# dome272/Paella

Measured on AMD Instinct MI355X. Metric: images/sec (whole node) + single-image ms, 256x256 @ 8 steps, higher is better.
Workload: dtype f32; 1 GPU; BASELINE configs[1]: Paella 573M-class (stand-in blocks=[4,8,4]) (570.3M params), 32x32 tokens = 256 px, 8 steps, CFG 8.0, CLIP-H-text only (S=4), batch 1 per GPU, + VQGAN f8 decode; denoiser=570m, sample_steps=8, noise=philox, submission=hip-graph replay, world_size_observed=1

## Files before the change

paella_amd/_lib.py:

```python
import ctypes
import os
from ctypes import POINTER, Structure, c_char, c_char_p, c_float, c_int, c_int32, c_int64, c_size_t, c_uint64, c_void_p

_HERE = os.path.dirname(os.path.abspath(__file__))
LIB_PATH = os.path.join(_HERE, "csrc", "libpaella_hip.so")

MAX_LEVELS = 8
MAX_BLOCK_TYPES = 8
ABI_VERSION = 8


class UnetConfig(Structure):
    _fields_ = [
        ("c_in", c_int32), ("c_out", c_int32), ("num_labels", c_int32), ("c_r", c_int32), ("patch_size", c_int32),
        ("c_cond", c_int32), ("n_levels", c_int32),
        ("c_hidden", c_int32 * MAX_LEVELS), ("nhead", c_int32 * MAX_LEVELS), ("blocks", c_int32 * MAX_LEVELS),
        ("level_config", (c_char * MAX_BLOCK_TYPES) * MAX_LEVELS),
        ("clip_embd", c_int32), ("byt5_embd", c_int32), ("clip_seq_len", c_int32), ("kernel_size", c_int32),
        ("self_attn", c_int32),
    ]


class VqganConfig(Structure):
    _fields_ = [
# ... 214 lines not shown
    "paella_test_gemm_dma": (c_int, [c_int]),
    "paella_test_gemm_epi_specialise": (c_int, [c_int]),
    "paella_test_gemm_raster": (c_int, [c_int]),
    "paella_test_gemm_ring": (c_int, [c_int]),
    "paella_test_ring_resident": (ctypes.c_long, [c_int, c_int]),
    "paella_test_gemm_site": (c_int, [c_int, c_int, c_int, c_int, c_int, c_int]),
    "paella_test_gemm_site_cfg": (c_int, [c_int, c_int, c_int, c_int, c_int, c_int, c_int]),
    "paella_test_gemm_big_stagger": (c_int, [c_int]),
    "paella_test_grn_fuse": (c_int, [c_int]),
    "paella_test_ln_fold_ratio": (c_int, [c_float]),
    "paella_test_ln_guard_counter": (c_int, [c_void_p]),
    "paella_test_mlp_grn_fused": (c_int, [c_void_p] * 10 + [c_int, c_int, c_int, c_void_p, c_size_t, c_void_p]),
    "paella_test_gemm_tail_tile": (c_int, [c_int]),
    "paella_test_tail_scores": (c_int, [c_void_p, c_void_p, c_int64, c_int, c_float, c_float, c_float, c_uint64, c_uint64, c_int64, c_void_p, c_void_p]),
    "paella_test_tail_scores_req": (c_int, [c_void_p, c_void_p, c_int64, c_int, c_void_p, c_void_p, c_void_p, c_int, c_uint64, c_void_p, c_void_p]),
    "paella_test_tail_filter_keep": (c_int, [c_void_p, c_void_p, c_int64, c_int, c_float, c_float, c_float, c_int, c_float, c_float, c_int, c_void_p, c_void_p, c_void_p,
                                             c_int, c_void_p, c_void_p, c_void_p, c_void_p, c_void_p]),
    "paella_test_renoise_scores": (c_int, [c_void_p, c_void_p, c_void_p, c_int64, c_int, c_uint64, c_uint64, c_int64, c_float, c_int, c_float, c_void_p, c_void_p, c_void_p,
                                           c_void_p, c_void_p, c_void_p, c_void_p, c_void_p, c_void_p, c_void_p, c_void_p, c_void_p]),
    "paella_test_gemm_prologue": (c_int, [c_void_p, c_void_p, c_void_p, c_int, c_int, c_int, c_int, c_void_p, c_void_p, c_int, c_void_p, c_int, c_int,
                                          c_void_p, c_size_t, c_void_p]),
    "paella_test_gemm_desc": (c_int, [POINTER(TestGemmArgs), c_int, c_int, c_void_p, c_size_t, c_void_p]),
    "paella_test_gemm_args_size": (c_size_t, []),
}

_lib = None


class PaellaHipError(RuntimeError):
    pass


def load():
    global _lib
    if _lib is not None:
        return _lib
    if not os.path.exists(LIB_PATH):
        raise PaellaHipError(
            "libpaella_hip.so is not built (%s). Run `python -m paella_amd.build` (needs hipcc); "
            "paella_amd has no non-HIP fallback." % LIB_PATH)
    try:
        lib = ctypes.CDLL(LIB_PATH)
    except OSError as e:
        raise PaellaHipError("cannot load %s: %s" % (LIB_PATH, e)) from e
    for name, (res, args) in list(SIGNATURES.items()) + list(TEST_HOOKS.items()):
        fn = getattr(lib, name)
# ... 41 lines not shown
```

paella_amd/csrc/common.h:

```cpp
#pragma once
#include <hip/hip_runtime.h>
#include <stdint.h>
#include <stddef.h>

typedef float f32x4 __attribute__((ext_vector_type(4)));

#define PAELLA_OK 0
#define PAELLA_ERR_ARG -1
#define PAELLA_ERR_HIP -2
#define PAELLA_ERR_WORKSPACE -3
#define PAELLA_ERR_STATE -4

void paella_set_error(const char* fmt, ...);

#define HIP_CHECK_RET(expr)                                                          \
    do {                                                                             \
        hipError_t _e = (expr);                                                      \
        if (_e != hipSuccess) {                                                      \
            paella_set_error("%s:%d: %s -> %s", __FILE__, __LINE__, #expr,           \
                             hipGetErrorString(_e));                                 \
            return PAELLA_ERR_HIP;                                                   \
        }                                                                            \
    } while (0)

// ... 128 lines not shown
int gemm_grn_fused_tile(int M, int C4, int C, int rows_per_sample, bool allow_64);
int gemm_tail_tiles_n(int M, int N, bool bf16_operands = false);
int launch_gemm_tail(const GemmArgs& g, hipStream_t stream);
int gemm_tail_config(int M, int N, bool bf16_operands = false);
int launch_tail_finalize(const TailArgs& a, const float* part_score, const int* part_idx, int tiles_n, hipStream_t stream);
static inline bool gemm_bf16_ok(int K, int lda, int ldw) { return K > 0 && (K & 63) == 0 && (lda & 7) == 0 && (ldw & 7) == 0; }

int launch_ln_rowstat_finalize(const float* stats, int nblk, int K, float eps, float* out4, int64_t M, const float* A32, unsigned short* A16, int lda, float ratio,
                               unsigned* guard_count, hipStream_t stream);

int launch_layernorm(const float* x, float* y, int64_t rows, int C, float eps, float g_mul, float g_add,
                     int s2d, int H, int W, hipStream_t stream);
int launch_layernorm16(const float* x, float* y, unsigned short* y16, int64_t rows, int C, float eps, float g_mul, float g_add,
                       int s2d, int H, int W, hipStream_t stream);
int launch_grn_apply16(unsigned short* h, const float* scale, const float* shift, int64_t rows, int rows_per_sample, int C, hipStream_t stream);
int launch_grn_partials_apply16(const float* part, const float* gamma, const float* shift, float* scale, unsigned short* h, int B, int rows_per_sample, int C, hipStream_t stream);
int launch_f32_to_bf16(const float* src, unsigned short* dst, size_t n, hipStream_t stream);
int launch_rowsum_bf16(const unsigned short* W, float* out, int N, int K, hipStream_t stream);

int launch_dwconv_ln(const float* x, const float* skip, const float* w, const float* bias, float* y,
                     int B, int H, int W, int C, float eps, hipStream_t stream, unsigned short* y16 = nullptr);
int launch_dwconv_res(const float* x, const float* xt, const float* w, const float* bias, float* y,
                      int B, int H, int W, int C, float gamma2, hipStream_t stream);

int launch_grn_scale(const float* g, const float* gamma, float* scale, float* tmp_gx, int B,
                     int rows_per_sample, int C, hipStream_t stream);

int launch_grn_from_partials(const float* part, const float* gamma, float* scale, int B, int groups, int C, hipStream_t stream);

int launch_embed_ln_unshuffle(const int64_t* tokens, const float* table, float* out, int B, int H, int W,
                              int c_in, int patch, int num_labels, float eps, hipStream_t stream);

int launch_timestep(const float* r, const float* freqs, const float* Wcat, const float* bcat, float* ts,
                    int B, int c_r, int total, float max_positions, float* r_embed_out, int reps, hipStream_t stream);
int launch_scale_shift(float* x, const float* ts, int ts_stride, int64_t rows, int rows_per_sample, int C,
                       hipStream_t stream);

int launch_silu(const float* x, float* y, int64_t n, hipStream_t stream);
int launch_copy_rows(const float* src, int lds, float* dst, int ldd, int64_t rows, int cols, hipStream_t stream);
int launch_axpby(float* x, const float* y, float a, float b, int64_t n, hipStream_t stream);
int launch_axpby16(float* x, const float* y, float a, float b, int64_t n, unsigned short* x16, hipStream_t stream);
int launch_axpby16_req(float* x, const float* y, const float* ab, int B, int64_t per_sample, unsigned short* x16, hipStream_t stream);

struct AttnArgs {
    const float* q; int ldq;
    const float* k_self; const float* v_self; int ld_self;
    const float* k_cond; const float* v_cond; int ld_cond;
    float* out; int ldo;
    int B, nhead, D, Lq, Lself, Lcond;
    float scale;
    const float* key_weights;
    int n_kw;
    unsigned short* out16;
    const unsigned short* q16; const unsigned short* k_self16; const unsigned short* v_self16; int ld16;
    const int* cond_len;
    const float* kw_table = nullptr;
    const int* kw_len = nullptr;
    int kw_pitch = 0;
    const int* q_groups = nullptr;
    const int* k_groups = nullptr;
    int qg_pitch = 0, kg_pitch = 0;
};
int launch_attention(const AttnArgs& a, hipStream_t stream);

struct TailArgs {
// ... 69 lines not shown
```

paella_amd/csrc/elementwise.hip:

```cpp
#include "common.h"
#include "gemm_device.h"

#define WAVES_PER_BLOCK 4

__device__ __forceinline__ float wave_sum(float v) {
#pragma unroll
    for (int o = 32; o > 0; o >>= 1) v += __shfl_xor(v, o, 64);
    return v;
}

__device__ __forceinline__ f32x4 ld4(const float* p) { return *reinterpret_cast<const f32x4*>(p); }
__device__ __forceinline__ void st4(float* p, f32x4 v) { *reinterpret_cast<f32x4*>(p) = v; }
__device__ __forceinline__ float hsum4(f32x4 v) { return (v[0] + v[1]) + (v[2] + v[3]); }
typedef __bf16 bf16x4 __attribute__((ext_vector_type(4)));
typedef __bf16 bf16x8 __attribute__((ext_vector_type(8)));
typedef float f32x8 __attribute__((ext_vector_type(8)));
__device__ __forceinline__ void st4h(unsigned short* p, f32x4 v) { *reinterpret_cast<bf16x4*>(p) = __builtin_convertvector(v, bf16x4); }

template <int NV>
__device__ __forceinline__ void ln_regs(f32x4 (&v)[NV], int C4, int lane, int C, float eps, float mul, float add) {
    float s = 0.f;
#pragma unroll
    for (int i = 0; i < NV; ++i)
        if (lane + i * 64 < C4) s += hsum4(v[i]);
// ... 158 lines not shown
                if (c4 < C4) acc[i] += ld4(xt + npos * C + c4 * 4) * ld4(w + tap * C + c4 * 4);
            }
        }
    }
#pragma unroll
    for (int i = 0; i < NV; ++i) {
        const int c4 = lane + i * 64;
        if (c4 < C4) st4(y + pos * C + c4 * 4, ld4(x + pos * C + c4 * 4) + acc[i] * gamma2);
    }
}

int launch_dwconv_res(const float* x, const float* xt, const float* w, const float* bias, float* y, int B, int H,
                      int W, int C, float gamma2, hipStream_t st) {
    const int64_t total = (int64_t)B * H * W;
    if (total <= 0) return PAELLA_OK;
    if (C & 3) { paella_set_error("dwconv_res: C %% 4 != 0"); return PAELLA_ERR_ARG; }
    const unsigned blocks = (unsigned)((total + WAVES_PER_BLOCK - 1) / WAVES_PER_BLOCK);
    DISPATCH_NV(C >> 2, hipLaunchKernelGGL((dwconv_res_kernel<NV>), dim3(blocks), dim3(64 * WAVES_PER_BLOCK), 0, st, x, xt, w,
                                           bias, y, B, H, W, C, gamma2));
    LAUNCH_CHECK_RET();
    return PAELLA_OK;
}

__global__ __launch_bounds__(256) void grn_sumsq_kernel(const float* __restrict__ g, float* __restrict__ gx, int rows_per_sample,
                                                        int C) {
    __shared__ float red[4][64];
    const int cl = threadIdx.x & 63, rg = threadIdx.x >> 6;
    const int c = blockIdx.x * 64 + cl;
    const int b = blockIdx.y;
    float s = 0.f;
    if (c < C) {
        const float* p = g + ((size_t)b * rows_per_sample) * C + c;
        for (int r = rg; r < rows_per_sample; r += 4) {
            const float v = p[(size_t)r * C];
            s += v * v;
        }
    }
    red[rg][cl] = s;
    __syncthreads();
    if (rg == 0 && c < C) gx[(size_t)b * C + c] = sqrtf((red[0][cl] + red[1][cl]) + (red[2][cl] + red[3][cl]));
}

__global__ __launch_bounds__(256) void grn_finalize_kernel(const float* __restrict__ gx, const float* __restrict__ gamma,
                                                           float* __restrict__ scale, int C) {
    __shared__ float red[256];
    const int b = blockIdx.x;
// ... 213 lines not shown
    int64_t blocks = (n + 255) / 256;
    if (blocks > 4096) blocks = 4096;
    hipLaunchKernelGGL(silu_kernel, dim3((unsigned)blocks), dim3(256), 0, st, x, y, n);
    LAUNCH_CHECK_RET();
    return PAELLA_OK;
}

__global__ __launch_bounds__(256) void copy_rows_kernel(const float* __restrict__ src, int lds_, float* __restrict__ dst, int ldd,
                                                        int64_t rows, int cols) {
    const int64_t total = rows * cols;
    for (int64_t i = (int64_t)blockIdx.x * 256 + threadIdx.x; i < total; i += (int64_t)gridDim.x * 256) {
        const int64_t r = i / cols;
        const int c = (int)(i - r * cols);
        dst[r * ldd + c] = src[r * lds_ + c];
    }
}
__global__ __launch_bounds__(256) void copy_rows4_kernel(const float* __restrict__ src, int lds_, float* __restrict__ dst, int ldd, unsigned total4, int cols4, FastDiv dC) {
    for (unsigned i = blockIdx.x * 256u + threadIdx.x; i < total4; i += gridDim.x * 256u) {
        const unsigned r = fast_div(i, dC);
        const unsigned c = (i - r * (unsigned)cols4) * 4u;
        st4(dst + (size_t)r * ldd + c, ld4(src + (size_t)r * lds_ + c));
    }
}
__global__ __launch_bounds__(256) void axpby_kernel(float* __restrict__ x, const float* __restrict__ y, float a, float b, int64_t n4, unsigned short* __restrict__ x16) {
    for (int64_t i = (int64_t)blockIdx.x * 256 + threadIdx.x; i < n4; i += (int64_t)gridDim.x * 256) {
        const f32x4 v = ld4(x + i * 4) * a + ld4(y + i * 4) * b;
        st4(x + i * 4, v);
        if (x16) st4h(x16 + i * 4, v);
    }
}
__global__ __launch_bounds__(256) void axpby_req_kernel(float* __restrict__ x, const float* __restrict__ y, const float* __restrict__ ab, int64_t per4, unsigned short* __restrict__ x16) {
    const int s = blockIdx.y;
    const float a = ab[2 * s], b = ab[2 * s + 1];
    for (int64_t j = (int64_t)blockIdx.x * 256 + threadIdx.x; j < per4; j += (int64_t)gridDim.x * 256) {
        const int64_t i = (int64_t)s * per4 + j;
        const f32x4 v = ld4(x + i * 4) * a + ld4(y + i * 4) * b;
        st4(x + i * 4, v);
        if (x16) st4h(x16 + i * 4, v);
    }
}
int launch_axpby16_req(float* x, const float* y, const float* ab, int B, int64_t per_sample, unsigned short* x16, hipStream_t st) {
    if (B <= 0 || per_sample <= 0) return PAELLA_OK;
    if (!ab || (per_sample & 3) || B > 65535) { paella_set_error("axpby_req: needs a pair table, per_sample %% 4 == 0 and at most 65535 samples"); return PAELLA_ERR_ARG; }
    int64_t blocks = (per_sample / 4 + 255) / 256;
    if (blocks > 1024) blocks = 1024;
    hipLaunchKernelGGL(axpby_req_kernel, dim3((unsigned)blocks, (unsigned)B), dim3(256), 0, st, x, y, ab, per_sample / 4, x16);
    LAUNCH_CHECK_RET();
    return PAELLA_OK;
}
int launch_axpby(float* x, const float* y, float a, float b, int64_t n, hipStream_t st) { return launch_axpby16(x, y, a, b, n, nullptr, st); }
int launch_axpby16(float* x, const float* y, float a, float b, int64_t n, unsigned short* x16, hipStream_t st) {
    if (n <= 0) return PAELLA_OK;
    if (n & 3) { paella_set_error("axpby: n %% 4 != 0"); return PAELLA_ERR_ARG; }
    int64_t blocks = (n / 4 + 255) / 256;
    if (blocks > 8192) blocks = 8192;
    hipLaunchKernelGGL(axpby_kernel, dim3((unsigned)blocks), dim3(256), 0, st, x, y, a, b, n / 4, x16);
    LAUNCH_CHECK_RET();
    return PAELLA_OK;
}

int launch_copy_rows(const float* src, int lds_, float* dst, int ldd, int64_t rows, int cols, hipStream_t st) {
    if (rows <= 0 || cols <= 0) return PAELLA_OK;
    if (!((cols | lds_ | ldd) & 3) && !(((uintptr_t)src | (uintptr_t)dst) & 15) && rows * (cols / 4) < 0x7fffffff) {
        const int64_t total4 = rows * (cols / 4);
        int64_t blocks4 = (total4 + 255) / 256;
        if (blocks4 > 4096) blocks4 = 4096;
        hipLaunchKernelGGL(copy_rows4_kernel, dim3((unsigned)blocks4), dim3(256), 0, st, src, lds_, dst, ldd, (unsigned)total4, cols / 4, fast_div_of((unsigned)(cols / 4)));
        LAUNCH_CHECK_RET();
        return PAELLA_OK;
    }
    int64_t blocks = (rows * cols + 255) / 256;
    if (blocks > 4096) blocks = 4096;
    hipLaunchKernelGGL(copy_rows_kernel, dim3((unsigned)blocks), dim3(256), 0, st, src, lds_, dst, ldd, rows, cols);
    LAUNCH_CHECK_RET();
    return PAELLA_OK;
}

__global__ __launch_bounds__(256) void grn_apply16_kernel(unsigned short* __restrict__ h, const float* __restrict__ scale, const float* __restrict__ shift,
                                                          unsigned total8, int C8, FastDiv dC8, FastDiv dRps) {
    for (unsigned i = blockIdx.x * 256u + threadIdx.x; i < total8; i += gridDim.x * 256u) {
        const unsigned row = fast_div(i, dC8);
        const unsigned c = (i - row * (unsigned)C8) * 8u;
        const unsigned b = fast_div(row, dRps);
        const bf16x8 v = *reinterpret_cast<const bf16x8*>(h + (size_t)i * 8);
        const float* sp = scale + (size_t)b * ((size_t)C8 * 8) + c;
        const f32x4 s0 = ld4(sp), s1 = ld4(sp + 4), t0 = ld4(shift + c), t1 = ld4(shift + c + 4);
        const f32x8 f = __builtin_convertvector(v, f32x8);
        f32x8 o;
#pragma unroll
        for (int e = 0; e < 4; ++e) { o[e] = f[e] * s0[e] + t0[e]; o[4 + e] = f[4 + e] * s1[e] + t1[e]; }
        *reinterpret_cast<bf16x8*>(h + (size_t)i * 8) = __builtin_convertvector(o, bf16x8);
    }
}
__global__ __launch_bounds__(256) void grn_apply16_cols_kernel(unsigned short* __restrict__ h, const float* __restrict__ scale, const float* __restrict__ shift, int C, int rows_per_sample) {
    const int c = (blockIdx.x * 64 + (threadIdx.x & 63)) * 8;
    const int b = blockIdx.z;
// ... 141 lines not shown
```

paella_amd/csrc/model.hip:

```cpp
#include "internal.h"
#include "test_hooks.h"
#include "../../include/paella_hip.h"

#include <math.h>
#include <stdarg.h>
#include <stdio.h>
#include <string.h>

#include <map>
#include <string>
#include <vector>

static thread_local char g_err[2048] = "";
void paella_set_error(const char* fmt, ...) {
    va_list ap;
    va_start(ap, fmt);
    vsnprintf(g_err, sizeof(g_err), fmt, ap);
    va_end(ap);
}
extern "C" const char* paella_last_error(void) { return g_err; }
extern "C" int paella_abi_version(void) { return PAELLA_ABI_VERSION; }

int devbuf_alloc(DevBuf& b, size_t n) {
    if (b.p && b.n == n) return PAELLA_OK;
// ... 877 lines not shown
    }

    if (m->ts_total > 0)
        RET_IF(launch_timestep(r, m->freqs.p, m->ts_w.p, m->ts_b.p, f.ts, B, c.c_r, m->ts_total, 10000.0f, f.remb, Bfull / B, st));

    const int h0 = H / p, w0 = W / p;
    const int64_t n0 = (int64_t)B * h0 * w0;
    RET_IF(launch_embed_ln_unshuffle(tokens, T(m, "in_mapper.0.weight"), f.h, B, H, W, c.c_in, p, c.num_labels, 1e-6f, st));
    {
        GemmArgs g = gemm_args(f.h, c.c_in * p * p, T(m, "embedding.1.weight"), c.c_in * p * p, f.g, c.c_hidden[0], (int)n0, c.c_hidden[0], c.c_in * p * p);
        g.ep.bias = T(m, "embedding.1.bias");
        RET_IF(launch_gemm(g, f.splitk, kSplitKBudget, st));
        RET_IF(launch_layernorm(f.g, f.xl[0], n0, c.c_hidden[0], 1e-6f, 1.f, 0.f, 0, 0, 0, st));
    }

    float* x = f.xl[0];
    int h = h0, w = w0;
    for (size_t bi = 0; bi < m->down.size(); ++bi) {
        const Block& b = m->down[bi];
        if ((int)bi == split && B != Bfull) {
            const int reps = Bfull / B;
            int lvl = 0;
            for (size_t j = 0; j < bi; ++j) if (m->down[j].type == BT_DOWN) lvl = m->down[j].level;
            for (int rep = 1; rep < reps; ++rep) {
                for (int l = 0; l <= lvl; ++l) {
                    const int64_t rows_l = (int64_t)B * (h0 >> l) * (w0 >> l);
                    const int cl = c.c_hidden[l];
                    RET_IF(launch_copy_rows(f.xl[l], cl, f.xl[l] + (size_t)rep * rows_l * cl, cl, rows_l, cl, st));
                }
                const int64_t rows_c = (int64_t)B * h * w;
                const int sc = c.c_hidden[lvl] / 16 * 2;
                if (f.rowstat && c.c_hidden[lvl] % 16 == 0)
                    RET_IF(launch_copy_rows(f.rowstat, sc, f.rowstat + (size_t)rep * rows_c * sc, sc, rows_c, sc, st));
                if (f.x16 && c.c_hidden[lvl] % 8 == 0) {
                    const int c2 = c.c_hidden[lvl] / 2;
                    RET_IF(launch_copy_rows(reinterpret_cast<const float*>(f.x16), c2, reinterpret_cast<float*>(f.x16) + (size_t)rep * rows_c * c2, c2, rows_c, c2, st));
                }
            }
            B = Bfull; cx.B = Bfull;
        }
        switch (b.type) {
            case BT_DOWN: {
                const int64_t rows_in = (int64_t)B * h * w;
                const unsigned short* const w16 = ((4 * b.c_from) % 64) == 0 ? T16(m, b.prefix + ".1.weight") : nullptr;
                if (w16) RET_IF(launch_layernorm16(x, nullptr, f.h16, rows_in, b.c_from, 1e-6f, 1.f, 0.f, 1, h, w, st));
                else RET_IF(launch_layernorm(x, f.h, rows_in, b.c_from, 1e-6f, 1.f, 0.f, 1, h, w, st));
                h >>= 1; w >>= 1;
                GemmArgs g = gemm_args(f.h, 4 * b.c_from, T(m, b.prefix + ".1.weight"), 4 * b.c_from, f.xl[b.level], b.c_to, (int)(rows_in / 4), b.c_to, 4 * b.c_from);
                if (w16) { g.A16 = f.h16; g.W16 = w16; }
                g.ep.bias = T(m, b.prefix + ".1.bias");
                RET_IF(launch_gemm(g, f.splitk, kSplitKBudget, st));
                x = f.xl[b.level];
                break;
            }
            case BT_RES: case BT_FF: RET_IF(run_mlp_block(cx, b, x, nullptr, h, w)); break;
            case BT_ATTN: RET_IF(run_attn_block(cx, b, x, h, w)); break;
            case BT_TS:
                if (b.ts_standalone)
                    RET_IF(launch_scale_shift(x, f.ts + b.ts_offset, m->ts_total, (int64_t)B * h * w, h * w, b.c, st));
                break;
            default: break;
// ... 27 lines not shown
                if (b.ts_standalone)
                    RET_IF(launch_scale_shift(x, f.ts + b.ts_offset, m->ts_total, (int64_t)B * h * w, h * w, b.c, st));
                break;
            default: break;
        }
    }
    {
        const int p2 = p * p;
        const int64_t n0 = (int64_t)B * h0 * w0;
        GemmArgs g = gemm_args(f.h, c.c_hidden[0], T(m, "clf.1.weight"), c.c_hidden[0], f.g, c.c_out, (int)n0, c.c_out * p2, c.c_hidden[0]);
        const unsigned short* const wc16 = (c.c_hidden[0] % 64) == 0 ? T16(m, "clf.1.weight") : nullptr;
        if (m->clf_from_stats) {
            g.A = x; g.ln_stats = f.rowstat; g.ln_nblk = c.c_hidden[0] / 16; g.ln_eps = 1e-6f; g.ln_wsum = m->wsum.at("clf.1.weight").p;
            if (wc16) { g.A16 = f.x16; g.W16 = wc16; g.ln_wsum = m->wsum16.at("clf.1.weight").p; }
        } else if (wc16) {
            RET_IF(launch_layernorm16(x, nullptr, f.h16, n0, c.c_hidden[0], 1e-6f, 1.f, 0.f, 0, 0, 0, st));
            g.A16 = f.h16; g.W16 = wc16;
        } else RET_IF(launch_layernorm(x, f.h, n0, c.c_hidden[0], 1e-6f, 1.f, 0.f, 0, 0, 0, st));
        g.ep.bias = T(m, "clf.1.bias");
        if (p == 2) { g.ep.store_mode = STORE_D2S; g.ep.sH = h0; g.ep.sW = w0; g.ep.sC = c.c_out; g.ep.n_seg_x = 2; }
        RET_IF(launch_gemm(g, f.splitk, kSplitKBudget, st));
        int64_t nt = (int64_t)B * H * W;
        const unsigned short* const wh16 = (c.c_out % 64) == 0 ? T16(m, "out_mapper.1.weight") : nullptr;
        if (wh16 && !mix) RET_IF(launch_layernorm16(f.g, nullptr, f.h16, nt, c.c_out, 1e-6f, 1.f, 0.f, 0, 0, 0, st));
        else RET_IF(launch_layernorm(f.g, f.h, nt, c.c_out, 1e-6f, 1.f, 0.f, 0, 0, 0, st));
        if (mix) {
            nt /= 2;
            if (mix_pairs) RET_IF(launch_axpby16_req(f.h, f.h + (size_t)nt * c.c_out, mix_pairs, n_unique, (int64_t)H * W * c.c_out, wh16 ? f.h16 : nullptr, st));
            else RET_IF(launch_axpby16(f.h, f.h + (size_t)nt * c.c_out, mix_c, mix_u, nt * c.c_out, wh16 ? f.h16 : nullptr, st));
        }
        GemmArgs go = gemm_args(f.h, c.c_out, T(m, "out_mapper.1.weight"), c.c_out, logits_out, c.num_labels, (int)nt, c.num_labels, c.c_out);
        if (wh16) { go.A16 = f.h16; go.W16 = wh16; }
        if (!tail) {
            RET_IF(launch_gemm_cfg(go, gemm_tail_config((int)nt, c.num_labels, wh16 != nullptr), 1, f.splitk, kSplitKBudget, st));
        } else {
            const int tn = gemm_tail_tiles_n((int)nt, c.num_labels, wh16 != nullptr);
            if (tn > (c.num_labels + 63) / 64) { paella_set_error("internal: fused tail tiles narrower than 64 labels (tiles_n=%d)", tn); return PAELLA_ERR_STATE; }
            if (tail->rows != nt || tail->L != c.num_labels) { paella_set_error("fused tail: row / label count mismatch"); return PAELLA_ERR_ARG; }
            go.C = nullptr;
            go.ft.temperature = tail->temperature; go.ft.mode = tail->mode; go.ft.seed = tail->seed; go.ft.seed_ptr = tail->seed_ptr;
            go.ft.offset = tail->offset; go.ft.row_offset = tail->row_offset; go.ft.row_offset_ptr = tail->row_offset_ptr;
            go.rq = tail->rq;
            go.ft.part_score = f.g;
            go.ft.part_idx = reinterpret_cast<int*>(f.g + (size_t)nt * tn);
            RET_IF(launch_gemm_tail(go, st));
            RET_IF(launch_tail_finalize(*tail, go.ft.part_score, go.ft.part_idx, tn, st));
        }
    }
    return PAELLA_OK;
}

static int run_step_block(const char* who, paella_unet* m, const paella_step_args& s, int need, void* ws, size_t ws_bytes, void* stream) {
    if ((!s.tail && !s.logits_out) || ((need & kNeedPairs) && !s.mix_pairs)) { paella_set_error("%s: null argument (logits_out / mix_pairs)", who); return PAELLA_ERR_ARG; }
// ... 337 lines not shown
    g.ep.bias = bias; g.ep.act = act; g.ep.residual = residual; g.ep.ldr = N; g.ep.c16 = C16;
    if (ln_stats) {
        static DevBuf wsum;
        if (wsum.n < (size_t)N) RET_IF(devbuf_alloc(wsum, (size_t)N));
        RET_IF(launch_rowsum_bf16(W16, wsum.p, N, K, (hipStream_t)stream));
        g.ln_stats = ln_stats; g.ln_nblk = K / 16; g.ln_eps = 1e-6f; g.ln_wsum = wsum.p;
    }
    return launch_gemm_cfg(g, tile_cfg, splitk, ws, ws_bytes, (hipStream_t)stream);
}
extern "C" int paella_test_gemm_bf16_ln(const unsigned short* A16, const float* A32, const unsigned short* W16, float* C, int M, int N, int K, const float* ln_stats,
                                        int tile_cfg, int splitk, void* ws, size_t ws_bytes, void* stream) {
    if (!ln_stats) { paella_set_error("gemm_bf16_ln: statistics required"); return PAELLA_ERR_ARG; }
    GemmArgs g = gemm_args(A32, K, nullptr, K, C, N, M, N, K);
    g.A16 = A16; g.W16 = W16;
    static DevBuf wsum;
    if (wsum.n < (size_t)N) RET_IF(devbuf_alloc(wsum, (size_t)N));
    RET_IF(launch_rowsum_bf16(W16, wsum.p, N, K, (hipStream_t)stream));
    g.ln_stats = ln_stats; g.ln_nblk = K / 16; g.ln_eps = 1e-6f; g.ln_wsum = wsum.p;
    return launch_gemm_cfg(g, tile_cfg, splitk, ws, ws_bytes, (hipStream_t)stream);
}
extern "C" int paella_test_grn_apply16(unsigned short* h, const float* scale, const float* shift, int64_t rows, int rows_per_sample, int C, void* stream) {
    return launch_grn_apply16(h, scale, shift, rows, rows_per_sample, C, (hipStream_t)stream);
}
extern "C" int paella_op_layernorm(const float* x, float* y, int64_t rows, int C, float eps, void* stream) {
    return launch_layernorm(x, y, rows, C, eps, 1.f, 0.f, 0, 0, 0, (hipStream_t)stream);
}
extern "C" int paella_op_dwconv_ln(const float* x, const float* skip, const float* w, const float* bias, float* y, int B, int H, int W,
                                   int C, float eps, void* stream) {
    return launch_dwconv_ln(x, skip, w, bias, y, B, H, W, C, eps, (hipStream_t)stream);
}
extern "C" int paella_op_grn_scale(const float* g, const float* gamma, float* scale, float* tmp, int B, int rows_per_sample, int C,
                                   void* stream) {
    return launch_grn_scale(g, gamma, scale, tmp, B, rows_per_sample, C, (hipStream_t)stream);
}
static int op_attention_impl(const float* q, const float* k_self, const float* v_self, const float* k_cond, const float* v_cond, float* out, int B, int nhead, int D,
                             int Lq, int Lself, int Lcond, const int* cond_len, const float* key_weights, int n_kw, KwTable kw, void* stream,
                             RgTable rg = {nullptr, 0, nullptr, 0}) {
    AttnArgs a;
    const int ld = nhead * D;
    a.q = q; a.ldq = ld; a.k_self = k_self; a.v_self = v_self; a.ld_self = ld; a.k_cond = k_cond; a.v_cond = v_cond; a.ld_cond = ld;
    a.out = out; a.ldo = ld; a.B = B; a.nhead = nhead; a.D = D; a.Lq = Lq; a.Lself = Lself; a.Lcond = Lcond;
    a.scale = 1.0f / sqrtf((float)D); a.key_weights = key_weights; a.n_kw = key_weights ? n_kw : 0; a.out16 = nullptr;
    a.q16 = nullptr; a.k_self16 = nullptr; a.v_self16 = nullptr; a.ld16 = 0; a.cond_len = cond_len;
    a.kw_table = kw.table; a.kw_len = kw.len; a.kw_pitch = kw.pitch;
    a.q_groups = rg.q; a.qg_pitch = rg.q_pitch; a.k_groups = rg.k; a.kg_pitch = rg.k_pitch;
    return launch_attention(a, (hipStream_t)stream);
// ... 48 lines not shown
```

paella_amd/csrc/vqmodel.hip:

```cpp
#include "internal.h"
#include "../../include/paella_hip.h"

#include <math.h>
#include <stdio.h>

#include <map>
#include <string>
#include <vector>

enum VqOp { VQ_CONV1, VQ_RES, VQ_CONV4S2, VQ_CONVT4, VQ_LATENT_BN };

struct VqBlock {
    VqOp op;
    int c_in, c_out;
    std::string prefix;
    float gam[6];
    DevBuf phase_w[4];
};

struct VqSpec { Repack kind; std::vector<int64_t> shape; bool is_int = false; };

struct paella_vqgan {
    paella_vqgan_config cfg;
    std::vector<int> c_levels;
// ... 212 lines not shown

struct VqBuffers { float *x, *t, *g, *a, *lat, *qe, *splitk; unsigned short *t16, *g16; };

static void vq_carve(const paella_vqgan* v, Arena& a, int B, int h, int w, VqBuffers& f) {
    f.splitk = a.take(kSplitKBudget / sizeof(float));
    const int L = v->cfg.levels;
    size_t xmax = 0, amax = 0;
    for (int i = 0; i < L; ++i) {
        const size_t rows = (size_t)B * (h << (L - 1 - i)) * (w << (L - 1 - i));
        const size_t n = rows * v->c_levels[i];
        if (n > xmax) xmax = n;
        if (i + 1 < L) {
            const size_t r1 = (size_t)B * (h << (L - 2 - i)) * (w << (L - 2 - i));
            const size_t a1 = r1 * 4 * v->c_levels[i + 1], a2 = r1 * 16 * v->c_levels[i];
            if (a1 > amax) amax = a1;
            if (a2 > amax) amax = a2;
        }
    }
    const size_t img_rows = (size_t)B * (h << (L - 1)) * (w << (L - 1));
    if (img_rows * 12 > amax) amax = img_rows * 12;
    f.x = a.take(xmax);
    f.t = a.take(xmax);
    f.g = a.take(4 * xmax);
    f.a = a.take(amax ? amax : 4);
    f.lat = a.take((size_t)B * h * w * v->cfg.c_latent);
    f.qe = a.take((size_t)B * h * w * v->cfg.c_latent);
    f.t16 = f.g16 = nullptr;
    if (v->precision == 1) {
        f.t16 = reinterpret_cast<unsigned short*>(a.take(xmax / 2 + 64));
        f.g16 = reinterpret_cast<unsigned short*>(a.take(2 * xmax + 64));
    }
}

extern "C" size_t paella_vqgan_workspace_bytes(const paella_vqgan* v, int B, int h, int w) {
    if (!v) return 0;
    VqBuffers f;
    Arena a(nullptr, 0);
    vq_carve(v, a, B, h, w, f);
    return a.off + 256;
}

static int vq_resblock(const paella_vqgan* v, const VqBlock& b, VqBuffers& f, int B, int h, int w, hipStream_t st) {
    const int c = b.c_in;
    const int64_t rows = (int64_t)B * h * w;
    RET_IF(launch_layernorm(f.x, f.t, rows, c, 1e-6f, 1.0f + b.gam[0], b.gam[1], 0, 0, 0, st));
    RET_IF(launch_dwconv_res(f.x, f.t, VT(v, b.prefix + ".depthwise.1.weight"), VT(v, b.prefix + ".depthwise.1.bias"), f.x, B, h, w, c,
                             b.gam[2], st));
    const unsigned short* const w1_16 = VT16(v, b.prefix + ".channelwise.0.weight");
    const unsigned short* const w2_16 = VT16(v, b.prefix + ".channelwise.2.weight");
    if (w1_16 && w2_16 && f.t16 && (c % 64) == 0) {
        RET_IF(launch_layernorm16(f.x, nullptr, f.t16, rows, c, 1e-6f, 1.0f + b.gam[3], b.gam[4], 0, 0, 0, st));
        GemmArgs g1 = gemm_args(nullptr, c, VT(v, b.prefix + ".channelwise.0.weight"), c, nullptr, 4 * c, (int)rows, 4 * c, c);
        g1.A16 = f.t16; g1.W16 = w1_16;
        g1.ep.bias = VT(v, b.prefix + ".channelwise.0.bias");
        g1.ep.act = ACT_GELU;
        g1.ep.c16 = f.g16;
        RET_IF(launch_gemm(g1, f.splitk, kSplitKBudget, st));
        GemmArgs g2 = gemm_args(nullptr, 4 * c, VT(v, b.prefix + ".channelwise.2.weight"), 4 * c, f.x, c, (int)rows, c, 4 * c);
        g2.A16 = f.g16; g2.W16 = w2_16;
        g2.ep.bias = VT(v, b.prefix + ".channelwise.2.bias");
        g2.ep.alpha = b.gam[5];
        g2.ep.residual = f.x; g2.ep.ldr = c;
        RET_IF(launch_gemm(g2, f.splitk, kSplitKBudget, st));
        return PAELLA_OK;
    }
    RET_IF(launch_layernorm(f.x, f.t, rows, c, 1e-6f, 1.0f + b.gam[3], b.gam[4], 0, 0, 0, st));
    GemmArgs g1 = gemm_args(f.t, c, VT(v, b.prefix + ".channelwise.0.weight"), c, f.g, 4 * c, (int)rows, 4 * c, c);
    g1.ep.bias = VT(v, b.prefix + ".channelwise.0.bias");
    g1.ep.act = ACT_GELU;
    RET_IF(launch_gemm(g1, f.splitk, kSplitKBudget, st));
    GemmArgs g2 = gemm_args(f.g, 4 * c, VT(v, b.prefix + ".channelwise.2.weight"), 4 * c, f.x, c, (int)rows, c, 4 * c);
    g2.ep.bias = VT(v, b.prefix + ".channelwise.2.bias");
    g2.ep.alpha = b.gam[5];
    g2.ep.residual = f.x; g2.ep.ldr = c;
    RET_IF(launch_gemm(g2, f.splitk, kSplitKBudget, st));
    return PAELLA_OK;
}

static int vq_run_decoder(paella_vqgan* v, VqBuffers& f, int B, int h, int w, float* img_out, hipStream_t st) {
    int ch = h, cw = w;
    const float* in = f.lat;
    for (VqBlock& b : v->dec) {
        const int64_t rows = (int64_t)B * ch * cw;
        switch (b.op) {
            case VQ_CONV1: {
                GemmArgs g = gemm_args(in, b.c_in, VT(v, b.prefix + ".weight"), b.c_in, f.x, b.c_out, (int)rows, b.c_out, b.c_in);
                g.ep.bias = VT(v, b.prefix + ".bias");
                RET_IF(launch_gemm(g, f.splitk, kSplitKBudget, st));
                break;
            }
            case VQ_RES: RET_IF(vq_resblock(v, b, f, B, ch, cw, st)); break;
            case VQ_CONVT4: {
                for (int ph = 0; ph < 4; ++ph) {
                    const int py = ph >> 1, px = ph & 1;
                    const bool implicit = (b.c_in & 31) == 0;
                    if (!implicit) RET_IF(launch_convT4_gather(f.x, f.a, B, ch, cw, b.c_in, py, px, st));
                    GemmArgs g = gemm_args(implicit ? f.x : f.a, 4 * b.c_in, b.phase_w[ph].p, 4 * b.c_in, f.t, b.c_out, (int)rows, b.c_out, 4 * b.c_in);
// ... 146 lines not shown
```

Measured before the change: 47.30 images/sec.

## Fuse VQGAN resblock LN+dwconv+LN, head LN+CFG mix, and batch replica copies

Fuses the VQGAN resblock front (layernorm, depthwise 3x3 conv with residual, second layernorm) into one kernel. Each wave recomputes the neighbour-row layernorms per tap instead of materialising the normalised tensor. The denoiser head layernorm and the CFG cond/uncond mix become a single kernel. The per-level replica copies before the batched block are merged into one multi-segment copy launch. The aim is fewer launches and fewer full-tensor round trips through memory, at the cost of 9x redundant LN work per resblock position and an extra buffer for the new residual.

```diff
diff --git a/paella_amd/_lib.py b/paella_amd/_lib.py
--- a/paella_amd/_lib.py
+++ b/paella_amd/_lib.py
@@ -260,6 +260,10 @@
                                           c_void_p, c_size_t, c_void_p]),
     "paella_test_gemm_desc": (c_int, [POINTER(TestGemmArgs), c_int, c_int, c_void_p, c_size_t, c_void_p]),
     "paella_test_gemm_args_size": (c_size_t, []),
+    "paella_test_vq_front_fused": (c_int, [c_int]),
+    "paella_test_vq_res_front": (c_int, [c_void_p, c_void_p, c_void_p, POINTER(c_float), c_void_p, c_void_p, c_void_p, c_int, c_int, c_int, c_int, c_void_p]),
+    "paella_test_head_ln_mix": (c_int, [c_void_p, c_void_p, c_void_p, c_int64, c_int, c_float, c_float, c_void_p, c_int, c_int, c_void_p]),
+    "paella_test_copy_batch": (c_int, [POINTER(c_void_p), POINTER(c_void_p), POINTER(c_int64), c_int, c_void_p]),
 }
 
 _lib = None
diff --git a/paella_amd/csrc/common.h b/paella_amd/csrc/common.h
--- a/paella_amd/csrc/common.h
+++ b/paella_amd/csrc/common.h
@@ -174,6 +174,8 @@
                      int B, int H, int W, int C, float eps, hipStream_t stream, unsigned short* y16 = nullptr);
 int launch_dwconv_res(const float* x, const float* xt, const float* w, const float* bias, float* y,
                       int B, int H, int W, int C, float gamma2, hipStream_t stream);
+int launch_vq_res_front(const float* x, const float* w, const float* bias, float* xn, float* t, unsigned short* t16, int B, int H, int W, int C,
+                        float eps, float m0, float a0, float gamma2, float m1, float a1, hipStream_t stream);
 
 int launch_grn_scale(const float* g, const float* gamma, float* scale, float* tmp_gx, int B,
                      int rows_per_sample, int C, hipStream_t stream);
@@ -190,9 +192,20 @@
 
 int launch_silu(const float* x, float* y, int64_t n, hipStream_t stream);
 int launch_copy_rows(const float* src, int lds, float* dst, int ldd, int64_t rows, int cols, hipStream_t stream);
+constexpr int kCopySegs = 8;
+struct CopySegs { const float* src[kCopySegs]; float* dst[kCopySegs]; unsigned end4[kCopySegs]; unsigned total4; int n; };
+struct CopyBatch {
+    CopySegs s;
+    hipStream_t st;
+    explicit CopyBatch(hipStream_t stream) : s{}, st(stream) {}
+    int add(const float* src, float* dst, int64_t n);
+    int flush();
+};
 int launch_axpby(float* x, const float* y, float a, float b, int64_t n, hipStream_t stream);
 int launch_axpby16(float* x, const float* y, float a, float b, int64_t n, unsigned short* x16, hipStream_t stream);
 int launch_axpby16_req(float* x, const float* y, const float* ab, int B, int64_t per_sample, unsigned short* x16, hipStream_t stream);
+int launch_head_ln_mix(const float* g, float* y, unsigned short* y16, int64_t rows, int C, float eps, float a, float b, const float* ab, int rows_per_sample,
+                       hipStream_t stream);
 
 struct AttnArgs {
     const float* q; int ldq;
diff --git a/paella_amd/csrc/elementwise.hip b/paella_amd/csrc/elementwise.hip
--- a/paella_amd/csrc/elementwise.hip
+++ b/paella_amd/csrc/elementwise.hip
@@ -204,6 +204,68 @@
     return PAELLA_OK;
 }
 
+template <int NV>
+__global__ __launch_bounds__(64 * WAVES_PER_BLOCK) void vq_res_front_kernel(const float* __restrict__ x, const float* __restrict__ w,
+                                                                           const float* __restrict__ bias, float* __restrict__ xn,
+                                                                           float* __restrict__ t, unsigned short* __restrict__ t16, int B, int H,
+                                                                           int W, int C, float eps, float m0, float a0, float gamma2, float m1,
+                                                                           float a1) {
+    const int lane = threadIdx.x & 63;
+    const int64_t pos = (int64_t)blockIdx.x * WAVES_PER_BLOCK + (threadIdx.x >> 6);
+    const int64_t total = (int64_t)B * H * W;
+    if (pos >= total) return;
+    const int C4 = C >> 2;
+    const int xx = (int)(pos % W);
+    const int yy = (int)((pos / W) % H);
+    const int64_t base = pos - (int64_t)yy * W - xx;
+    int co[NV];
+    f32x4 acc[NV], v[NV];
+#pragma unroll
+    for (int i = 0; i < NV; ++i) {
+        co[i] = min(lane + i * 64, C4 - 1) * 4;
+        acc[i] = ld4(bias + co[i]);
+    }
+#pragma unroll(NV <= 2 ? 9 : 1)
+    for (int tap = 0; tap < 9; ++tap) {
+        const int ky = tap / 3, kx = tap - ky * 3;
+        const int sy = min(max(yy + ky - 1, 0), H - 1);
+        const int sx = min(max(xx + kx - 1, 0), W - 1);
+        const int64_t npos = base + (int64_t)sy * W + sx;
+#pragma unroll
+        for (int i = 0; i < NV; ++i) v[i] = ld4(x + npos * C + co[i]);
+        ln_regs<NV>(v, C4, lane, C, eps, m0, a0);
+#pragma unroll
+        for (int i = 0; i < NV; ++i) acc[i] += v[i] * ld4(w + tap * C + co[i]);
+    }
+#pragma unroll
+    for (int i = 0; i < NV; ++i) {
+        v[i] = ld4(x + pos * C + co[i]) + acc[i] * gamma2;
+        if (lane + i * 64 < C4) st4(xn + pos * C + co[i], v[i]);
+    }
+    ln_regs<NV>(v, C4, lane, C, eps, m1, a1);
+#pragma unroll
+    for (int i = 0; i < NV; ++i) {
+        const int c4 = lane + i * 64;
+        if (c4 < C4) {
+            if (t16) st4h(t16 + pos * C + c4 * 4, v[i]);
+            else st4(t + pos * C + c4 * 4, v[i]);
+        }
+    }
+}
+
+int launch_vq_res_front(const float* x, const float* w, const float* bias, float* xn, float* t, unsigned short* t16, int B, int H, int W, int C,
+                        float eps, float m0, float a0, float gamma2, float m1, float a1, hipStream_t st) {
+    const int64_t total = (int64_t)B * H * W;
+    if (total <= 0) return PAELLA_OK;
+    if (C <= 0 || (C & 3)) { paella_set_error("vq_res_front: C must be a positive multiple of 4 (C=%d)", C); return PAELLA_ERR_ARG; }
+    if (!x || !xn || xn == x || (!t && !t16)) { paella_set_error("vq_res_front: needs x, a separate xn and one of t / t16"); return PAELLA_ERR_ARG; }
+    const unsigned blocks = (unsigned)((total + WAVES_PER_BLOCK - 1) / WAVES_PER_BLOCK);
+    DISPATCH_NV(C >> 2, hipLaunchKernelGGL((vq_res_front_kernel<NV>), dim3(blocks), dim3(64 * WAVES_PER_BLOCK), 0, st, x, w, bias, xn, t, t16, B,
+                                           H, W, C, eps, m0, a0, gamma2, m1, a1));
+    LAUNCH_CHECK_RET();
+    return PAELLA_OK;
+}
+
 __global__ __launch_bounds__(256) void grn_sumsq_kernel(const float* __restrict__ g, float* __restrict__ gx, int rows_per_sample,
                                                         int C) {
     __shared__ float red[4][64];
@@ -463,9 +525,22 @@
         st4(dst + (size_t)r * ldd + c, ld4(src + (size_t)r * lds_ + c));
     }
 }
+__global__ __launch_bounds__(256) void copy_segs_kernel(CopySegs s) {
+    for (unsigned i = blockIdx.x * 256u + threadIdx.x; i < s.total4; i += gridDim.x * 256u) {
+        const float* sp = s.src[0];
+        float* dp = s.dst[0];
+        unsigned start = 0;
+#pragma unroll
+        for (int j = 0; j + 1 < kCopySegs; ++j)
+            if (j + 1 < s.n && i >= s.end4[j]) { sp = s.src[j + 1]; dp = s.dst[j + 1]; start = s.end4[j]; }
+        const size_t o = (size_t)(i - start) * 4u;
+        st4(dp + o, ld4(sp + o));
+    }
+}
+__device__ __forceinline__ f32x4 mix4(f32x4 x, f32x4 y, float a, float b) { return x * a + y * b; }
 __global__ __launch_bounds__(256) void axpby_kernel(float* __restrict__ x, const float* __restrict__ y, float a, float b, int64_t n4, unsigned short* __restrict__ x16) {
     for (int64_t i = (int64_t)blockIdx.x * 256 + threadIdx.x; i < n4; i += (int64_t)gridDim.x * 256) {
-        const f32x4 v = ld4(x + i * 4) * a + ld4(y + i * 4) * b;
+        const f32x4 v = mix4(ld4(x + i * 4), ld4(y + i * 4), a, b);
         st4(x + i * 4, v);
         if (x16) st4h(x16 + i * 4, v);
     }
@@ -475,10 +550,51 @@
     const float a = ab[2 * s], b = ab[2 * s + 1];
     for (int64_t j = (int64_t)blockIdx.x * 256 + threadIdx.x; j < per4; j += (int64_t)gridDim.x * 256) {
         const int64_t i = (int64_t)s * per4 + j;
-        const f32x4 v = ld4(x + i * 4) * a + ld4(y + i * 4) * b;
+        const f32x4 v = mix4(ld4(x + i * 4), ld4(y + i * 4), a, b);
         st4(x + i * 4, v);
         if (x16) st4h(x16 + i * 4, v);
     }
+}
+template <int NV>
+__global__ __launch_bounds__(64 * WAVES_PER_BLOCK) void head_ln_mix_kernel(const float* __restrict__ g, float* __restrict__ y, unsigned short* __restrict__ y16,
+                                                                          int64_t rows, int C, float eps, float g_mul, float g_add, float a, float b,
+                                                                          const float* __restrict__ ab, int rows_per_sample) {
+    const int lane = threadIdx.x & 63;
+    const int64_t row = (int64_t)blockIdx.x * WAVES_PER_BLOCK + (threadIdx.x >> 6);
+    if (row >= rows) return;
+    const int C4 = C >> 2;
+    f32x4 vc[NV], vu[NV];
+#pragma unroll
+    for (int i = 0; i < NV; ++i) {
+        const int co = min(lane + i * 64, C4 - 1) * 4;
+        vc[i] = ld4(g + row * C + co);
+        vu[i] = ld4(g + (row + rows) * C + co);
+    }
+    if (ab) {
+        const int64_t s = row / rows_per_sample;
+        a = ab[2 * s]; b = ab[2 * s + 1];
+    }
+    ln_regs<NV>(vc, C4, lane, C, eps, g_mul, g_add);
+    ln_regs<NV>(vu, C4, lane, C, eps, g_mul, g_add);
+#pragma unroll
+    for (int i = 0; i < NV; ++i) {
+        const int c4 = lane + i * 64;
+        if (c4 < C4) {
+            const f32x4 v = mix4(vc[i], vu[i], a, b);
+            st4(y + row * C + c4 * 4, v);
+            if (y16) st4h(y16 + row * C + c4 * 4, v);
+        }
+    }
+}
+int launch_head_ln_mix(const float* g, float* y, unsigned short* y16, int64_t rows, int C, float eps, float a, float b, const float* ab,
+                       int rows_per_sample, hipStream_t st) {
+    if (rows <= 0) return PAELLA_OK;
+    if (C <= 0 || (C & 3) || !g || !y || g == y || (ab && rows_per_sample <= 0)) { paella_set_error("head_ln_mix: needs C a positive multiple of 4, separate g and y, and rows per sample with a pair table"); return PAELLA_ERR_ARG; }
+    const unsigned blocks = (unsigned)((rows + WAVES_PER_BLOCK - 1) / WAVES_PER_BLOCK);
+    DISPATCH_NV(C >> 2, hipLaunchKernelGGL((head_ln_mix_kernel<NV>), dim3(blocks), dim3(64 * WAVES_PER_BLOCK), 0, st, g, y, y16, rows, C, eps, 1.f, 0.f,
+                                           a, b, ab, rows_per_sample));
+    LAUNCH_CHECK_RET();
+    return PAELLA_OK;
 }
 int launch_axpby16_req(float* x, const float* y, const float* ab, int B, int64_t per_sample, unsigned short* x16, hipStream_t st) {
     if (B <= 0 || per_sample <= 0) return PAELLA_OK;
@@ -513,6 +629,31 @@
     int64_t blocks = (rows * cols + 255) / 256;
     if (blocks > 4096) blocks = 4096;
     hipLaunchKernelGGL(copy_rows_kernel, dim3((unsigned)blocks), dim3(256), 0, st, src, lds_, dst, ldd, rows, cols);
+    LAUNCH_CHECK_RET();
+    return PAELLA_OK;
+}
+
+int CopyBatch::add(const float* src, float* dst, int64_t n) {
+    if (n <= 0) return PAELLA_OK;
+    if ((n & 3) || (((uintptr_t)src | (uintptr_t)dst) & 15) || n / 4 >= 0x40000000) {
+        if (n >= 0x7fffffff) { paella_set_error("copy: range of %lld floats too long", (long long)n); return PAELLA_ERR_ARG; }
+        return launch_copy_rows(src, (int)n, dst, (int)n, 1, (int)n, st);
+    }
+    if (s.n == kCopySegs || (uint64_t)s.total4 + (uint64_t)(n / 4) >= 0x7fffffffull) {
+        const int rc = flush();
+        if (rc != PAELLA_OK) return rc;
+    }
+    s.src[s.n] = src; s.dst[s.n] = dst;
+    s.total4 += (unsigned)(n / 4);
+    s.end4[s.n++] = s.total4;
+    return PAELLA_OK;
+}
+int CopyBatch::flush() {
+    if (s.n == 0) return PAELLA_OK;
+    unsigned blocks = (s.total4 + 255u) / 256u;
+    if (blocks > 4096u) blocks = 4096u;
+    hipLaunchKernelGGL(copy_segs_kernel, dim3(blocks), dim3(256), 0, st, s);
+    s.n = 0; s.total4 = 0;
     LAUNCH_CHECK_RET();
     return PAELLA_OK;
 }
diff --git a/paella_amd/csrc/model.hip b/paella_amd/csrc/model.hip
--- a/paella_amd/csrc/model.hip
+++ b/paella_amd/csrc/model.hip
@@ -923,21 +923,23 @@
             const int reps = Bfull / B;
             int lvl = 0;
             for (size_t j = 0; j < bi; ++j) if (m->down[j].type == BT_DOWN) lvl = m->down[j].level;
+            CopyBatch cp(st);
             for (int rep = 1; rep < reps; ++rep) {
                 for (int l = 0; l <= lvl; ++l) {
                     const int64_t rows_l = (int64_t)B * (h0 >> l) * (w0 >> l);
                     const int cl = c.c_hidden[l];
-                    RET_IF(launch_copy_rows(f.xl[l], cl, f.xl[l] + (size_t)rep * rows_l * cl, cl, rows_l, cl, st));
+                    RET_IF(cp.add(f.xl[l], f.xl[l] + (size_t)rep * rows_l * cl, rows_l * cl));
                 }
                 const int64_t rows_c = (int64_t)B * h * w;
                 const int sc = c.c_hidden[lvl] / 16 * 2;
                 if (f.rowstat && c.c_hidden[lvl] % 16 == 0)
-                    RET_IF(launch_copy_rows(f.rowstat, sc, f.rowstat + (size_t)rep * rows_c * sc, sc, rows_c, sc, st));
+                    RET_IF(cp.add(f.rowstat, f.rowstat + (size_t)rep * rows_c * sc, rows_c * sc));
                 if (f.x16 && c.c_hidden[lvl] % 8 == 0) {
                     const int c2 = c.c_hidden[lvl] / 2;
-                    RET_IF(launch_copy_rows(reinterpret_cast<const float*>(f.x16), c2, reinterpret_cast<float*>(f.x16) + (size_t)rep * rows_c * c2, c2, rows_c, c2, st));
+                    RET_IF(cp.add(reinterpret_cast<const float*>(f.x16), reinterpret_cast<float*>(f.x16) + (size_t)rep * rows_c * c2, rows_c * c2));
                 }
             }
+            RET_IF(cp.flush());
             B = Bfull; cx.B = Bfull;
         }
         switch (b.type) {
@@ -1011,13 +1013,11 @@
         RET_IF(launch_gemm(g, f.splitk, kSplitKBudget, st));
         int64_t nt = (int64_t)B * H * W;
         const unsigned short* const wh16 = (c.c_out % 64) == 0 ? T16(m, "out_mapper.1.weight") : nullptr;
-        if (wh16 && !mix) RET_IF(launch_layernorm16(f.g, nullptr, f.h16, nt, c.c_out, 1e-6f, 1.f, 0.f, 0, 0, 0, st));
-        else RET_IF(launch_layernorm(f.g, f.h, nt, c.c_out, 1e-6f, 1.f, 0.f, 0, 0, 0, st));
         if (mix) {
             nt /= 2;
-            if (mix_pairs) RET_IF(launch_axpby16_req(f.h, f.h + (size_t)nt * c.c_out, mix_pairs, n_unique, (int64_t)H * W * c.c_out, wh16 ? f.h16 : nullptr, st));
-            else RET_IF(launch_axpby16(f.h, f.h + (size_t)nt * c.c_out, mix_c, mix_u, nt * c.c_out, wh16 ? f.h16 : nullptr, st));
-        }
+            RET_IF(launch_head_ln_mix(f.g, f.h, wh16 ? f.h16 : nullptr, nt, c.c_out, 1e-6f, mix_c, mix_u, mix_pairs, H * W, st));
+        } else if (wh16) RET_IF(launch_layernorm16(f.g, nullptr, f.h16, nt, c.c_out, 1e-6f, 1.f, 0.f, 0, 0, 0, st));
+        else RET_IF(launch_layernorm(f.g, f.h, nt, c.c_out, 1e-6f, 1.f, 0.f, 0, 0, 0, st));
         GemmArgs go = gemm_args(f.h, c.c_out, T(m, "out_mapper.1.weight"), c.c_out, logits_out, c.num_labels, (int)nt, c.num_labels, c.c_out);
         if (wh16) { go.A16 = f.h16; go.W16 = wh16; }
         if (!tail) {
@@ -1401,6 +1401,21 @@
 extern "C" int paella_test_grn_apply16(unsigned short* h, const float* scale, const float* shift, int64_t rows, int rows_per_sample, int C, void* stream) {
     return launch_grn_apply16(h, scale, shift, rows, rows_per_sample, C, (hipStream_t)stream);
 }
+extern "C" int paella_test_head_ln_mix(const float* g, float* y, unsigned short* y16, int64_t rows, int C, float a, float b, const float* ab, int rows_per_sample,
+                                       int fused, void* stream) {
+    hipStream_t st = (hipStream_t)stream;
+    if (fused) return launch_head_ln_mix(g, y, y16, rows, C, 1e-6f, a, b, ab, rows_per_sample, st);
+    if (ab && (rows_per_sample <= 0 || rows % rows_per_sample)) { paella_set_error("head_ln_mix: rows must be whole samples"); return PAELLA_ERR_ARG; }
+    RET_IF(launch_layernorm(g, y, 2 * rows, C, 1e-6f, 1.f, 0.f, 0, 0, 0, st));
+    if (ab) return launch_axpby16_req(y, y + (size_t)rows * C, ab, (int)(rows / rows_per_sample), (int64_t)rows_per_sample * C, y16, st);
+    return launch_axpby16(y, y + (size_t)rows * C, a, b, rows * C, y16, st);
+}
+extern "C" int paella_test_copy_batch(const float* const* src, float* const* dst, const int64_t* n, int count, void* stream) {
+    if (count < 0 || (count && (!src || !dst || !n))) { paella_set_error("copy_batch: null argument"); return PAELLA_ERR_ARG; }
+    CopyBatch cp((hipStream_t)stream);
+    for (int i = 0; i < count; ++i) RET_IF(cp.add(src[i], dst[i], n[i]));
+    return cp.flush();
+}
 extern "C" int paella_op_layernorm(const float* x, float* y, int64_t rows, int C, float eps, void* stream) {
     return launch_layernorm(x, y, rows, C, eps, 1.f, 0.f, 0, 0, 0, (hipStream_t)stream);
 }
diff --git a/paella_amd/csrc/vqmodel.hip b/paella_amd/csrc/vqmodel.hip
--- a/paella_amd/csrc/vqmodel.hip
+++ b/paella_amd/csrc/vqmodel.hip
@@ -1,5 +1,6 @@
 #include "internal.h"
 #include "../../include/paella_hip.h"
+#include "test_hooks.h"
 
 #include <math.h>
 #include <stdio.h>
@@ -258,6 +259,7 @@
     f.x = a.take(xmax);
     f.t = a.take(xmax);
     f.g = a.take(4 * xmax);
+    if (xmax > amax) amax = xmax;
     f.a = a.take(amax ? amax : 4);
     f.lat = a.take((size_t)B * h * w * v->cfg.c_latent);
     f.qe = a.take((size_t)B * h * w * v->cfg.c_latent);
@@ -276,16 +278,33 @@
     return a.off + 256;
 }
 
+static int g_vq_front_fused = 1;
+extern "C" int paella_test_vq_front_fused(int on) { g_vq_front_fused = on ? 1 : 0; return PAELLA_OK; }
+
+static int vq_res_front(const float* x, const float* w, const float* bias, const float* gam, float* xn, float* t, unsigned short* t16, int B, int h, int wd,
+                        int c, hipStream_t st) {
+    if (g_vq_front_fused)
+        return launch_vq_res_front(x, w, bias, xn, t16 ? nullptr : t, t16, B, h, wd, c, 1e-6f, 1.0f + gam[0], gam[1], gam[2], 1.0f + gam[3], gam[4], st);
+    const int64_t rows = (int64_t)B * h * wd;
+    RET_IF(launch_layernorm(x, t, rows, c, 1e-6f, 1.0f + gam[0], gam[1], 0, 0, 0, st));
+    RET_IF(launch_dwconv_res(x, t, w, bias, xn, B, h, wd, c, gam[2], st));
+    return launch_layernorm16(xn, t16 ? nullptr : t, t16, rows, c, 1e-6f, 1.0f + gam[3], gam[4], 0, 0, 0, st);
+}
+extern "C" int paella_test_vq_res_front(const float* x, const float* w, const float* bias, const float* gam5, float* xn, float* t, unsigned short* t16, int B,
+                                        int H, int W, int C, void* stream) {
+    if (!x || !w || !bias || !gam5 || !xn || !t || xn == x) { paella_set_error("vq_res_front: null argument, or xn == x"); return PAELLA_ERR_ARG; }
+    return vq_res_front(x, w, bias, gam5, xn, t, t16, B, H, W, C, (hipStream_t)stream);
+}
+
 static int vq_resblock(const paella_vqgan* v, const VqBlock& b, VqBuffers& f, int B, int h, int w, hipStream_t st) {
     const int c = b.c_in;
     const int64_t rows = (int64_t)B * h * w;
-    RET_IF(launch_layernorm(f.x, f.t, rows, c, 1e-6f, 1.0f + b.gam[0], b.gam[1], 0, 0, 0, st));
-    RET_IF(launch_dwconv_res(f.x, f.t, VT(v, b.prefix + ".depthwise.1.weight"), VT(v, b.prefix + ".depthwise.1.bias"), f.x, B, h, w, c,
-                             b.gam[2], st));
     const unsigned short* const w1_16 = VT16(v, b.prefix + ".channelwise.0.weight");
     const unsigned short* const w2_16 = VT16(v, b.prefix + ".channelwise.2.weight");
-    if (w1_16 && w2_16 && f.t16 && (c % 64) == 0) {
-        RET_IF(launch_layernorm16(f.x, nullptr, f.t16, rows, c, 1e-6f, 1.0f + b.gam[3], b.gam[4], 0, 0, 0, st));
+    const bool fast = w1_16 && w2_16 && f.t16 && (c % 64) == 0;
+    float* const xn = g_vq_front_fused ? f.a : f.x;
+    RET_IF(vq_res_front(f.x, VT(v, b.prefix + ".depthwise.1.weight"), VT(v, b.prefix + ".depthwise.1.bias"), b.gam, xn, f.t, fast ? f.t16 : nullptr, B, h, w, c, st));
+    if (fast) {
         GemmArgs g1 = gemm_args(nullptr, c, VT(v, b.prefix + ".channelwise.0.weight"), c, nullptr, 4 * c, (int)rows, 4 * c, c);
         g1.A16 = f.t16; g1.W16 = w1_16;
         g1.ep.bias = VT(v, b.prefix + ".channelwise.0.bias");
@@ -296,11 +315,10 @@
         g2.A16 = f.g16; g2.W16 = w2_16;
         g2.ep.bias = VT(v, b.prefix + ".channelwise.2.bias");
         g2.ep.alpha = b.gam[5];
-        g2.ep.residual = f.x; g2.ep.ldr = c;
+        g2.ep.residual = xn; g2.ep.ldr = c;
         RET_IF(launch_gemm(g2, f.splitk, kSplitKBudget, st));
         return PAELLA_OK;
     }
-    RET_IF(launch_layernorm(f.x, f.t, rows, c, 1e-6f, 1.0f + b.gam[3], b.gam[4], 0, 0, 0, st));
     GemmArgs g1 = gemm_args(f.t, c, VT(v, b.prefix + ".channelwise.0.weight"), c, f.g, 4 * c, (int)rows, 4 * c, c);
     g1.ep.bias = VT(v, b.prefix + ".channelwise.0.bias");
     g1.ep.act = ACT_GELU;
@@ -308,7 +326,7 @@
     GemmArgs g2 = gemm_args(f.g, 4 * c, VT(v, b.prefix + ".channelwise.2.weight"), 4 * c, f.x, c, (int)rows, c, 4 * c);
     g2.ep.bias = VT(v, b.prefix + ".channelwise.2.bias");
     g2.ep.alpha = b.gam[5];
-    g2.ep.residual = f.x; g2.ep.ldr = c;
+    g2.ep.residual = xn; g2.ep.ldr = c;
     RET_IF(launch_gemm(g2, f.splitk, kSplitKBudget, st));
     return PAELLA_OK;
 }
```

After: 47.51 images/sec (median of 6 runs). About the same (+0.4%).
